# dsforza96/yocto-hair

Measured on AMD Instinct MI355X. Metric: Msamples/sec (whole node), 720x720x1536spp sphere-hairblock; per-pixel L2 vs CPU ref, higher is better.
Workload: dtype f32

## Files before the change

### include/yhair.h

```cpp
#ifndef YHAIR_H_
#define YHAIR_H_

#include <stdint.h>

#ifdef __cplusplus
extern "C" {
#endif

#define YH_OK 0
#define YH_E_INVALID -1
#define YH_E_DEVICE -2
#define YH_E_STATE -3
#define YH_E_IO -4
#define YH_E_SELFTEST -5


typedef struct yh_shape {
  int          num_vertices;
  const float* positions;
  const float* normals;
  const float* radius;
  int          num_lines;
  const int*   lines;
  int          num_triangles;
// ... 123 lines not shown
int yh_unpack_tiles_device(yh_context* ctx, const void* device_packed,
    int src_rank, int world, void* device_image);
int64_t yh_shard_pixels(const yh_context* ctx, int rank, int world);

int yh_gather_framebuffer(yh_context** contexts, int n, float* rgba);

int yh_download_rng(yh_context* ctx, uint64_t* state_inc);

int yh_trace_samples_counted(yh_context* ctx, int nsamples, yh_workcounts* out);

int yh_last_trace_ms(const yh_context* ctx, float* ms, int* launches);

int yh_launch_shape(const yh_context* ctx);
int yh_kernel_trials(const yh_context* ctx, double* ms_per_sample, int* trials, int count);
int yh_trials_pending(const yh_context* ctx);
int         yh_set_trial_cache_dir(const char* dir);
const char* yh_default_trial_cache_dir(void);

int yh_tile_costs(yh_context* ctx, uint32_t* ticks, int count);
int yh_item_costs(yh_context* ctx, uint32_t* costs, int count);


#define YH_HAIR_BRDF_FLOATS 30

enum {
  YH_LOBE_DIFFUSE            = 0,
  YH_LOBE_SPECULAR           = 1,
  YH_LOBE_METAL              = 2,
  YH_LOBE_TRANSMISSION       = 3,
  YH_LOBE_REFRACTION         = 4,
// ... 54 lines not shown
```

### yocto-hair_amd/csrc/dev_items.h

```cpp
#ifndef YH_DEV_ITEMS_H_
#define YH_DEV_ITEMS_H_
#include "dev_path.h"

using namespace yhd;

#define YH_BLOCK 512
#define YH_MIN_WAVES 4

#define YH_QUADS (YH_BLOCK / 4)
template <bool COUNT, bool GENERAL, int BLOCK, int SHADER, int MODE = YH_MODE_QUAD>
YH_DEV void trace_items(const yhd_scene& sc, const yhd_state& st, int nsamples, yhd_counters* counters, unsigned int block = blockIdx.x,
    unsigned int blocks = gridDim.x) {
  constexpr int LPP    = YH_IS_HEX(MODE) ? 16 : YH_IS_OCT(MODE) ? 8 : 4;
  constexpr int GROUPS = BLOCK / LPP;
  extern __shared__ v4f lds_dyn[];
  YH_LDS unsigned int* lds_stack = (YH_LDS unsigned int*)lds_dyn;
  YH_LDS v4f*          lds_tabs  = (YH_LDS v4f*)(lds_stack + ((MODE == YH_MODE_QUAD ? sc.stack_entries : YH_IS_HEX(MODE) ? sc.stack_entries16 : sc.stack_entries8) + YH_HITROWS) * GROUPS);
  trace_ctx tc;
  tc.sc = &sc;
  tc.ls = nullptr, tc.sc_dev = nullptr;
  YH_LDS float* lds_cam;
  stage_tables(sc, lds_tabs, threadIdx.x, blockDim.x, tc, lds_cam);
  __syncthreads();

  tc.lds_stack = lds_stack + (threadIdx.x / LPP);
  stats_t stats = {};
  tc.stats = COUNT ? &stats : nullptr;

  const int lane = threadIdx.x & 63;
  const int by_position = (int)(blocks * (BLOCK / 64));
  int       t_first     = __builtin_amdgcn_readfirstlane((int)(block * (BLOCK / 64) + (threadIdx.x >> 6)));
  while (true) {
    int t = t_first;
    if (t < 0) {
      if (lane == 0) t = atomicAdd(st.tile_cursor, 1);
      t = __builtin_amdgcn_readfirstlane(t) + by_position;
    }
    t_first = -1;
    if (t >= st.num_tiles) break;
    unsigned long long t0 = wall_clock64();
    int  item  = st.tiles[t];
    int  half  = 0;
    if (YH_IS_OCT(MODE)) half = item & 1, item >>= 1;
    if (YH_IS_HEX(MODE)) half = item & 3, item >>= 2;
    int  tile  = item >> 2, part = item & 3;
    int  pq    = YH_IS_HEX(MODE) ? half * 4 + (lane >> 4) : YH_IS_OCT(MODE) ? half * 8 + (lane >> 3) : lane >> 2;
    int  i     = (tile % st.tiles_x) * YH_TILE + (part & 1) * 4 + (pq & 3);
    int  j     = (tile / st.tiles_x) * YH_TILE + (part >> 1) * 4 + (pq >> 2);
    bool owner = i < st.width && j < st.height;
    size_t pix = owner ? (size_t)j * st.width + i : 0;
    rng_t  rng;
    rng.state      = st.rng_state[pix];
    rng.inc        = st.rng_inc[pix];
    yhd_float4 acc = st.accum[pix];
    int    left    = owner ? nsamples : 0;
    bool   alive   = false;
    path_t ps;
    ps.bounce = 0, ps.hit = false;
    unsigned long long cyc_trace = 0, cyc_shade = 0;
    unsigned int       w_iters = 0, w_steps = 0, l_steps = 0, l_iters = 0;
    while (true) {
      if (!alive && left > 0) {
        yhd_camera cam;
        for (int k = 0; k < 12; k++) cam.frame[k] = lds_cam[k];
        cam.lens = lds_cam[12], cam.film_x = lds_cam[13], cam.film_y = lds_cam[14], cam.focus = lds_cam[15], cam.aperture = lds_cam[16];
        path_begin(cam, ps, rng, i, j, st.width, st.height);
        left--;
        alive = true;
      }
      if (!__any(alive)) break;
// ... 42 lines not shown
      }
      {
        unsigned int b[10] = {stats.t_node, stats.l_node, stats.t_line, stats.l_line, stats.t_tri, stats.l_tri, stats.t_enter,
            stats.l_enter, stats.t_scene, stats.l_scene};
        for (int k = 0; k < 10; k++) {
          for (int off = 32; off > 0; off >>= 1) b[k] += (unsigned int)__shfl_xor((int)b[k], off, 64);
          if (lane == 0) atomicAdd(&counters->branch[k], (unsigned long long)b[k]);
        }
      }
      stats = stats_t{};
    }
    if (owner && (lane & (LPP - 1)) == 0) {
      st.rng_state[pix] = rng.state;
      st.accum[pix]     = acc;
    }
    if (lane == 0) {
      unsigned int dt = (unsigned int)(wall_clock64() - t0);
      if (YH_IS_OCT(MODE) || YH_IS_HEX(MODE)) atomicAdd(&st.tile_cost[item], dt);
      else st.tile_cost[item] = dt;
      if (COUNT) atomicAdd(&counters->cyc_tile, (unsigned long long)dt);
    }
  }
}
typedef void (*trace_kernel_t)(const yhd_scene, const yhd_state, int, yhd_counters*);
#define YH_OCT_BLOCK 256
template <bool COUNT, bool GENERAL, int BLOCK, int WAVES, int MODE = YH_MODE_QUAD>
__global__ __launch_bounds__(BLOCK, WAVES) void k_trace(const yhd_scene sc, const yhd_state st,
    int nsamples, yhd_counters* counters) {
  trace_items<COUNT, GENERAL, BLOCK, YH_SHADER_PATH, MODE>(sc, st, nsamples, counters);
}
template <bool GENERAL>
__global__ __launch_bounds__(YH_BLOCK, YH_MIN_WAVES) void k_trace_sbs(const yhd_scene sc, const yhd_state st, int nsamples, int oct_blocks,
    int quad_items, int oct_entries) {
  if ((int)blockIdx.x < oct_blocks) {
    yhd_state so   = st;
    so.tiles       = st.tiles + quad_items, so.num_tiles = oct_entries, so.tile_cursor = st.tile_cursor + 16;
    trace_items<false, GENERAL, YH_BLOCK, YH_SHADER_PATH, YH_MODE_OCT>(sc, so, nsamples, nullptr, blockIdx.x, (unsigned)oct_blocks);
  } else {
    yhd_state sq = st;
    sq.num_tiles = quad_items;
    trace_items<false, GENERAL, YH_BLOCK, YH_SHADER_PATH, YH_MODE_QUAD>(sc, sq, nsamples, nullptr, blockIdx.x - (unsigned)oct_blocks, gridDim.x - (unsigned)oct_blocks);
  }
}
#endif
```

### yocto-hair_amd/csrc/yh_device.h

```cpp
#ifndef YH_DEVICE_H_
#define YH_DEVICE_H_
#include <stdint.h>

#define YH_KIND_LINES 1
#define YH_KIND_TRIANGLES 2
#define YH_TILE 8
#define YH_MAX_LIGHTS 16
#define YH_MAX_ENVS 4

typedef struct yhd_float4 { float x, y, z, w; } yhd_float4;
typedef struct yhd_int4 { int x, y, z, w; } yhd_int4;

typedef struct yhd_object {
  float frame[12];
  float inv_frame[12];
  int   kind;
  int   node_base;
  int   prim_base;
  int   vert_base;
  int   elem_base;
  int   has_normals;
  int   material;
  int   has_texcoords;
  float wbox_min[4], wbox_max[4];
// ... 96 lines not shown
  const yhd_float4* light_table;
  int               light_table_f4;
  int               scene_wide_root;
  const float*      env_tab;
  int               env_tab_light;
  int               env_tab_k, env_tab_stride;
  int               lds_materials;
  int               stack_entries8;
  int               stack_entries16;
  const yhd_float4* lane_blob;
  long long         lane_blob_units;
} yhd_scene;
#define YH_MATERIAL_F4 17
#define YHD_LDS_TABLES_F4(sc) ((sc)->lds_scene_f4 + 5 + (sc)->light_table_f4 + ((sc)->env_tab_k + 3) / 4 + YH_MATERIAL_F4 * (sc)->lds_materials)

typedef struct yhd_state {
  uint64_t*   rng_state;
  uint64_t*   rng_inc;
  yhd_float4* accum;
  const int*  tiles;
  int*        tile_cursor;
  int         num_groups;
  int         group_begin[9];
  unsigned int* tile_cost;
  int         num_tiles;
  int         shader;
  int         launch_shape;
  int         width, height;
  int         tiles_x;
  int         samples_done;
  int         bounces;
  float       clamp;
  int         shard_rank, shard_world;
} yhd_state;

enum yhd_shape {
  YH_SHAPE_QUAD       = 0,
  YH_SHAPE_QUAD_DENSE = 1,
  YH_SHAPE_RETIRED    = 2,
  YH_SHAPE_STREAM     = 3,
  YH_SHAPE_OCT        = 4,
  YH_SHAPE_SBS        = 5,
  YH_SHAPE_HEX        = 6,
  YH_SHAPE_OCT_PAIRS  = 7,
  YH_SHAPE_HEX_GROUPS = 8,
  YH_SHAPES
};
enum yhd_shape_kind { YH_SHAPE_KIND_QUAD, YH_SHAPE_KIND_WIDE, YH_SHAPE_KIND_STREAM, YH_SHAPE_KIND_SBS, YH_SHAPE_KIND_RETIRED };
// ... 55 lines not shown
```

### yocto-hair_amd/host/context.cpp

```cpp
#include "context_internal.h"

std::string g_create_error = "no error";

int fail(yh_context* ctx, int code, const char* fmt, ...) {
  char    buf[512];
  va_list ap;
  va_start(ap, fmt);
  vsnprintf(buf, sizeof(buf), fmt, ap);
  va_end(ap);
  if (ctx) ctx->error = buf;
  else g_create_error = buf;
  return code;
}

int upload(yh_context* ctx, DevBuf& buf, const void* src, size_t bytes) {
  YH_WAIT(ctx);
  buf.reset();
  size_t alloc = std::max<size_t>(bytes, 16);
  HIPCHK(ctx, hipMalloc(&buf.p, alloc));
  buf.bytes = alloc;
  if (bytes) HIPCHK(ctx, hipMemcpy(buf.p, src, bytes, hipMemcpyHostToDevice));
  return YH_OK;
}
int upload_keep(yh_context* ctx, DevBuf& buf, const void* src, size_t bytes) {
// ... 69 lines not shown
  (void)hipSetDevice(ctx->device);
  if (ctx->stream && wait_for_launch(ctx) != YH_OK) return;
  if (ctx->ev0) (void)hipEventDestroy(ctx->ev0);
  if (ctx->ev1) (void)hipEventDestroy(ctx->ev1);
  if (ctx->stream) (void)hipStreamDestroy(ctx->stream);
  delete ctx;
}

const char* yh_last_error(const yh_context* ctx) { return ctx ? ctx->error.c_str() : g_create_error.c_str(); }

int yh_set_shard(yh_context* ctx, int rank, int world) {
  if (!ctx) return YH_E_INVALID;
  if (world < 1 || rank < 0 || rank >= world) return fail(ctx, YH_E_INVALID, "bad shard %d of %d", rank, world);
  if (rank != ctx->rank || world != ctx->world) ctx->item_cost.clear();
  ctx->rank = rank, ctx->world = world;
  ctx->have_state = false;
  return YH_OK;
}

int yh_image_size(const yh_context* ctx, int* width, int* height) {
  if (!ctx || !ctx->have_state) return YH_E_STATE;
  if (width) *width = ctx->state.width;
  if (height) *height = ctx->state.height;
  return YH_OK;
}

int yh_download(yh_context* ctx, float* rgba) {
  if (!ctx || !rgba) return YH_E_INVALID;
  if (!ctx->have_state) return fail(ctx, YH_E_STATE, "yh_download before yh_init_state");
  HIPCHK(ctx, hipSetDevice(ctx->device));
  size_t bytes = (size_t)ctx->state.width * ctx->state.height * 16;
// ... 44 lines not shown
```

### yocto-hair_amd/host/context_internal.h

```cpp
#ifndef YH_CONTEXT_INTERNAL_H_
#define YH_CONTEXT_INTERNAL_H_
#include <hip/hip_runtime_api.h>
#include <dlfcn.h>
#include <fcntl.h>
#include <sys/stat.h>
#include <unistd.h>
#include <rccl/rccl.h>

#include <algorithm>
#include <chrono>
#include <cmath>
#include <cstdarg>
#include <cstddef>
#include <cstdio>
#include <cstdlib>
#include <cstring>
#include <limits>
#include <map>
#include <mutex>
#include <tuple>
#include <string>
#include <memory>
#include <thread>
#include <vector>
// ... 170 lines not shown
  bool        poisoned = false;
  bool      have_scene = false;
  yhd_scene scene{};
  DevBuf    d_prims, d_vpos, d_elems, d_objects, d_materials, d_scene_nodes,
      d_scene_prims, d_light_cdf, d_env_texels, d_light_table, d_env_tab;
  int       stack_need = 0, stack_need8 = 0, stack_need16 = 0;
  struct LaneShape { int kind, num_nodes, prim_base, num_prims; long long node_off, test_off, node_off8, node_off16; };
  std::vector<LaneShape>   lane_shapes;
  long long                lane_units = 0;
  DevBuf                   d_lane_blob;
  bool             have_state = false;
  yhd_state        state{};
  yh_trace_params  params{};
  DevBuf           d_textures, d_tex_texels, d_vtex, d_maps;
  DevBuf           d_rng_state, d_rng_inc, d_accum, d_tiles, d_image, d_counters, d_tile_cursor, d_tile_cost;
  std::vector<int> owned;
  std::vector<unsigned int>  item_cost;
  int              rank = 0, world = 1;
  int              num_tiles_total = 0;
  float            last_ms = 0;
  int              last_launches = 0;
  int              last_nsamples = 0;
  unsigned         launches_of_image = 0;
  int              launch_shape = YH_SHAPE_QUAD;
  int              last_shape = -1;
  bool             async_pending = false;
  bool             last_counted = false;
  DevBuf                  d_gather_send, d_gather_recv;
  std::vector<ncclComm_t> comms;
  std::vector<int>        comm_devices;
// ... 45 lines not shown
int upload(yh_context* ctx, DevBuf& buf, const void* src, size_t bytes);
int upload_keep(yh_context* ctx, DevBuf& buf, const void* src, size_t bytes);
int alloc_zero(yh_context* ctx, DevBuf& buf, size_t bytes);
yhd_float4 node_lo(const yhh::Node& n);
yhd_float4 node_hi(const yhh::Node& n);
int forced_shape();
void trials_load(yh_context* ctx);
bool trials_off();
void record_launch(yh_context* ctx, int nsamples, bool fresh_costs);
bool trial_pending(const yh_context* ctx);
int pick_launch_shape(const yh_context* ctx, int nsamples);
bool settle_launch_shape(yh_context* ctx, bool counted, int nsamples, bool sync);
void build_work_items(const yh_context* ctx, std::vector<int>& items);
void prepare_work_list(yh_context* ctx, std::vector<int>& items, int shape);
int upload_work_items(yh_context* ctx);
int expensive_items(const yh_context* ctx, const std::vector<int>& items);
bool side_by_side_grids(const yh_context* ctx, int* oct_blocks, int* quad_blocks);
void split_items_side_by_side(yh_context* ctx, std::vector<int>& items);
void lay_out_range(const yh_context* ctx, int* items, size_t n, int wpb, int G, int block_offset = 0);
int replan_after_launch(yh_context* ctx, int nsamples);
bool lane_kernels_can_address(const yh_context* ctx);
int stream_geometry(const yh_context* ctx, int num_items, int* slots_per_wave, int* grid_blocks, int* lds_out, bool* single_generation = nullptr);
void note_stream_wave_log(yh_context* ctx, const unsigned long long* log, size_t waves);
void deal_items_for_stream(yh_context* ctx, std::vector<int>& items);
int build_bvh_device(yh_context* ctx, const std::vector<yhh::Box>& boxes, yhh::Tree& tree);
int stream_impl(yh_context* ctx, int nsamples, bool sync);
int trace_impl(yh_context* ctx, int nsamples, bool counted, bool sync);
int wait_for_launch(yh_context* ctx);
int side_by_side_impl(yh_context* ctx, int nsamples, bool sync);
void destroy_communicators(yh_context* ctx);
// ... 5 lines not shown
```

### yocto-hair_amd/host/launch_plan.cpp

```cpp
#include "context_internal.h"

#include "build_id.h"

static bool dense_by_costs(const yh_context* ctx, bool* known, bool* chain_bound = nullptr, bool* chain16 = nullptr) {
  uint64_t sum = 0, mx = 0;
  for (int t : ctx->owned)
    for (int p = 0; p < 4; p++) {
      uint64_t c = ctx->item_cost[(size_t)t * 4 + p];
      sum += c, mx = std::max(mx, c);
    }
  *known = mx != 0;
  if (mx == 0) return false;
  static const double share = std::max(1, getenv("YHAIR_DEVICE_SHARE") ? atoi(getenv("YHAIR_DEVICE_SHARE")) : 1);
  int    lds      = yhk_trace_lds_bytes(&ctx->scene, YH_SHAPE_QUAD);
  double resident = (double)ctx->num_cus * std::max(1, yhk_trace_occupancy(lds, ctx->scene.general_materials, YH_SHAPE_QUAD)) * (yhk_block_threads(YH_SHAPE_QUAD) / 64) / share;
  if (getenv("YHAIR_TIMING")) fprintf(stderr, "[yhair] launch shape: worth %.0f items, resident waves %.0f\n", (double)sum / (double)mx, resident);
  if (chain_bound) {
    const int    lds4 = yhk_trace_lds_bytes(&ctx->scene, YH_SHAPE_OCT);
    const double res4 = (double)ctx->num_cus * std::max(1, yhk_trace_occupancy(lds4, ctx->scene.general_materials, YH_SHAPE_OCT)) * (yhk_block_threads(YH_SHAPE_OCT) / 64) / share;
    *chain_bound      = 2.0 * (double)sum / (double)mx <= 1.1 * res4;
    if (chain16) *chain16 = 4.0 * (double)sum / (double)mx <= 2.5 * res4;
  }
  return (double)sum / (double)mx >= resident;
}
// ... 235 lines not shown
    for (int p = 0; p < 4; p++) {
      unsigned item = (unsigned)(t * 4 + p);
      keys.push_back(((uint64_t)(0xFFFFFFFFu - ctx->item_cost[item]) << 32) | item);
    }
  if (!keys.empty()) {
    auto mid = keys.begin() + keys.size() / 2;
    std::nth_element(keys.begin(), mid, keys.end());
    uint64_t median_cost = 0xFFFFFFFFu - (uint32_t)(*mid >> 32);
    uint64_t cut_cost    = std::min<uint64_t>(0xFFFFFFFFu, median_cost * 8 + 1);
    uint64_t cut_key     = (uint64_t)(0xFFFFFFFFu - (uint32_t)cut_cost) << 32;
    auto heavy_end = std::partition(keys.begin(), keys.end(), [&](uint64_t k) { return k < cut_key; });
    std::sort(keys.begin(), heavy_end);
  }
  items.resize(keys.size());
  for (size_t i = 0; i < keys.size(); i++) items[i] = (int)(keys[i] & 0xFFFFFFFFu);
}

int expensive_items(const yh_context* ctx, const std::vector<int>& items) {
  if (items.empty()) return 0;
  const uint64_t top = ctx->item_cost[(size_t)items[0]];
  int n = 0;
  for (int it : items) {
    if ((uint64_t)ctx->item_cost[(size_t)it] * 5 < top || top == 0) break;
    n++;
  }
  return n;
}
bool side_by_side_grids(const yh_context* ctx, int* oct_blocks, int* quad_blocks) {
  const int lds = yhk_trace_sbs_lds_bytes(&ctx->scene), occ = yhk_trace_sbs_occupancy(lds, ctx->scene.general_materials);
  if (occ < 1) return false;
// ... 71 lines not shown
  if (forced_shape() < 0) {
    const int kind = yhd_shapes[shape].kind;
    int       P = 0, grid = 0;
    if ((kind == YH_SHAPE_KIND_STREAM && !stream_geometry(ctx, (int)ctx->owned.size() * 4, &P, &grid, nullptr)) ||
        (kind == YH_SHAPE_KIND_WIDE && !counted && yhk_trace_occupancy(yhk_trace_lds_bytes(&ctx->scene, shape), general, shape) < 1))
      ctx->shape_ms[shape] = std::numeric_limits<double>::infinity(), shape = fallback(shape);
  }
  if (shape == ctx->state.launch_shape) return false;
  ctx->launch_shape = ctx->state.launch_shape = shape;
  return true;
}

int replan_after_launch(yh_context* ctx, int nsamples) {
  const unsigned li      = ++ctx->launches_of_image;
  const bool     refresh = (li & (li - 1)) == 0 || ctx->last_ms >= 50.0f || (!ctx->costs_settled && nsamples >= YH_TRIAL_SPP && ctx->state.shader == YH_SHADER_PATH);
  if (refresh) HIPCHK(ctx, hipMemcpy(ctx->item_cost.data(), ctx->d_tile_cost.p, ctx->item_cost.size() * 4, hipMemcpyDeviceToHost));
  if (refresh) ctx->last_nsamples = nsamples;
  if (refresh && ctx->last_shape == YH_SHAPE_SBS)
    for (int it : ctx->hy_oct_items) ctx->item_cost[(size_t)it] = (unsigned int)((double)ctx->item_cost[(size_t)it] * (1.0 / 1.48));
  if (ctx->state.shader == YH_SHADER_PATH && (refresh || ctx->have_costs)) record_launch(ctx, nsamples, refresh);
  if (!refresh) return YH_OK;
  return upload_work_items(ctx);
}

bool lane_kernels_can_address(const yh_context* ctx) { return (long long)ctx->lane_units * 32ll <= 0xFFFFFE00ll; }

int stream_geometry(const yh_context* ctx, int num_items, int* slots_per_wave, int* grid_blocks, int* lds_out, bool* single_generation) {
  if (!lane_kernels_can_address(ctx)) return 0;
  const int     wpb    = yhk_stream_block_threads() / 64;
  const int64_t pixels = (int64_t)num_items * 16;
  int           P      = (int)std::max<int64_t>(128, std::min<int64_t>(192, (pixels / ((int64_t)ctx->num_cus * 16) + 63) / 64 * 64));
  const bool    forced = getenv("YHAIR_ST_SLOTS") != nullptr;
  if (forced) P = std::max(64, std::min(4096, atoi(getenv("YHAIR_ST_SLOTS")) / 64 * 64));
  int lds_bytes = yhk_stream_lds_bytes(YHD_LDS_TABLES_F4(&ctx->scene), P);
// ... 144 lines not shown
```

### yocto-hair_amd/host/scene_upload.cpp

```cpp
#include "context_internal.h"

#include <atomic>

static int dev_alloc(yh_context* ctx, DevBuf& buf, size_t bytes) {
  buf.reset();
  HIPCHK(ctx, hipMalloc(&buf.p, std::max<size_t>(bytes, 16)));
  buf.bytes = std::max<size_t>(bytes, 16);
  return YH_OK;
}

void make_material(const yh_material& m, yhd_material& d) {
  memset(&d, 0, sizeof(d));
  memcpy(d.emission, m.emission, 12);
  memcpy(d.color, m.color, 12);
  float dmax    = fmax_(fmax_(m.color[0], m.color[1]), m.color[2]);
  d.diffuse_pdf = dmax ? dmax / dmax : 0.0f;
  d.thin        = m.thin;
  d.specular = m.specular, d.metallic = m.metallic, d.roughness = m.roughness, d.ior = m.ior;
  d.transmission = m.transmission;
  d.opacity      = m.opacity * ((1.0f + 1.0f + 1.0f) / 3);
  if (d.opacity > 0.999f) d.opacity = 1;
  d.emission_tex = m.emission_tex - 1, d.color_tex = m.color_tex - 1, d.scattering_tex = m.scattering_tex - 1;
  d.trdepth = m.trdepth;
  d.plain = m.specular == 0 && m.metallic == 0 && m.transmission == 0 && d.opacity == 1 && m.emission_tex == 0 &&
// ... 110 lines not shown
  std::vector<yhd_int4>   elems;
  size_t total_prim_f4 = 0;
  for (int si = 0; si < sd->num_shapes; si++) {
    auto& s = sd->shapes[si];
    if (s.num_vertices <= 0 || !s.positions) return fail(ctx, YH_E_INVALID, "shape %d has no vertices", si);
    const bool lines = s.num_lines > 0;
    if (!lines && s.num_triangles <= 0) return fail(ctx, YH_E_INVALID, "shape %d has no lines or triangles", si);
    const int nel = lines ? s.num_lines : s.num_triangles;
    if (nel >= (1 << 27)) return fail(ctx, YH_E_INVALID, "shape %d has %d elements (limit %d)", si, nel, (1 << 27) - 1);
    info[si].kind = lines ? YH_KIND_LINES : YH_KIND_TRIANGLES, info[si].num_prims = nel, info[si].has_normals = s.normals != nullptr;
    info[si].prim_base = (int)total_prim_f4;
    total_prim_f4 += (size_t)nel * (lines ? 4 : 6);
  }
  if (total_prim_f4 > (size_t)std::numeric_limits<int>::max()) return fail(ctx, YH_E_INVALID, "scene too large for 32-bit record offsets (%zu primitive float4)", total_prim_f4);
  int rc;
  ctx->have_scene = false, ctx->have_state = false;
  ctx->scene.lane_blob = nullptr, ctx->scene.prims = nullptr;
  ctx->d_prims.reset(), ctx->d_lane_blob.reset();
  if ((rc = dev_alloc(ctx, ctx->d_prims, total_prim_f4 * 16))) return rc;
  lap("validation, record array");
  const char* bvh_env   = getenv("YHAIR_BVH");
  const bool  host_only = bvh_env && !strcmp(bvh_env, "host"), device_all = bvh_env && !strcmp(bvh_env, "device");
  for (int si = 0; si < sd->num_shapes; si++) {
    auto&      s     = sd->shapes[si];
    auto&      I     = info[si];
    const bool lines = I.kind == YH_KIND_LINES;
    const int  nel   = I.num_prims;
    const int* idx   = lines ? s.lines : s.triangles;
    {
      std::atomic<bool> bad{false};
      parallel_for(nel * (lines ? 2 : 3), [&](int k) {
// ... 492 lines not shown
```

### yocto-hair_amd/host/trace_launch.cpp

```cpp
#include "context_internal.h"

int wait_for_launch(yh_context* ctx) {
  if (ctx->poisoned) return fail(ctx, YH_E_DEVICE, "a launch of this context exceeded its deadline: the context refuses further work, destroy it");
  const double timeout = yhh::launch_timeout_s();
  const int    device  = ctx->device;
  hipStream_t  stream  = ctx->stream;
  int          e       = 0;
  const double spin_s  = std::min(std::min(0.050, timeout), 1.25e-3 * (double)ctx->last_ms + 0.001);
  {
    const auto t0 = std::chrono::steady_clock::now();
    while (true) {
      const hipError_t q = hipStreamQuery(stream);
      if (q == hipSuccess) return YH_OK;
      if (q != hipErrorNotReady) return fail(ctx, YH_E_DEVICE, "hipStreamQuery: %s", hipGetErrorString(q));
      if (std::chrono::duration<double>(std::chrono::steady_clock::now() - t0).count() > spin_s) break;
    }
  }
  const int    rc      = ctx->sync_call.run(
      [device, stream]() {
        hipError_t se = hipSetDevice(device);
        return (int)(se != hipSuccess ? se : hipStreamSynchronize(stream));
      },
      timeout, &e);
  if (rc == yhh::WAIT_EXPIRED) {
// ... 56 lines not shown
    ctx->have_costs = false, ctx->costs_settled = false, ctx->dense = -1, ctx->chain = -1, ctx->chain16 = -1, ctx->launch_shape = YH_SHAPE_QUAD;
    for (double& t : ctx->shape_ms) t = 0;
    for (int& t : ctx->shape_trials) t = 0;
    new_image = true;
  }
  std::vector<int> tiles;
  build_work_items(ctx, tiles);
  const int first_shape = forced_shape() >= 0 ? forced_shape() : ctx->launch_shape;
  prepare_work_list(ctx, tiles, params->shader == YH_SHADER_PATH ? first_shape : YH_SHAPE_QUAD);
  tiles.reserve(4 * (size_t)ctx->num_tiles_total * 4 + 4);
  int rc;
  if ((rc = upload(ctx, ctx->d_rng_state, st.data(), npix * 8))) return rc;
  if ((rc = upload(ctx, ctx->d_rng_inc, inc.data(), npix * 8))) return rc;
  if ((rc = alloc_zero(ctx, ctx->d_accum, npix * 16))) return rc;
  if ((rc = alloc_zero(ctx, ctx->d_image, npix * 16))) return rc;
  {
    const size_t n = tiles.size();
    tiles.resize(std::max(n, 4 * owned.size() * 4), 0);
    if ((rc = upload(ctx, ctx->d_tiles, tiles.data(), tiles.size() * 4))) return rc;
    tiles.resize(n);
  }
  if ((rc = alloc_zero(ctx, ctx->d_counters, sizeof(yhd_counters)))) return rc;
  if ((rc = alloc_zero(ctx, ctx->d_tile_cursor, 8 * 16 * 4))) return rc;
  if ((rc = alloc_zero(ctx, ctx->d_tile_cost, (size_t)ctx->num_tiles_total * 16))) return rc;
  auto& s = ctx->state;
  s.tile_cursor = (int*)ctx->d_tile_cursor.p, s.tile_cost = (unsigned int*)ctx->d_tile_cost.p;
  s.rng_state = (uint64_t*)ctx->d_rng_state.p, s.rng_inc = (uint64_t*)ctx->d_rng_inc.p;
  s.accum = (yhd_float4*)ctx->d_accum.p, s.tiles = (const int*)ctx->d_tiles.p;
  s.launch_shape = first_shape;
  s.num_tiles = (int)tiles.size(), s.width = w, s.height = h, s.tiles_x = tx;
  if (new_image || !same_work) ctx->launches_of_image = 0;
  s.samples_done = 0, s.bounces = params->bounces, s.clamp = params->clamp, s.shader = params->shader;
  s.shard_rank = ctx->rank, s.shard_world = ctx->world;
  ctx->have_state = true;
  lap("work list, buffers, copies");
  if (new_image) trials_load(ctx);
  bool measured = false;
  for (int t : owned)
    for (int q = 0; q < 4 && !measured; q++) measured = ctx->item_cost[(size_t)t * 4 + q] != 0;
  if (!measured && !owned.empty() && params->shader == YH_SHADER_PATH && !getenv("YHAIR_NO_PROBE")) {
    ctx->state.launch_shape = YH_SHAPE_QUAD;
    int prc = trace_impl(ctx, 1, false, true);
    if (prc) return prc;
    HIPCHK(ctx, hipMemcpy(ctx->d_rng_state.p, st.data(), npix * 8, hipMemcpyHostToDevice));
    HIPCHK(ctx, hipMemsetAsync(ctx->d_accum.p, 0, npix * 16, ctx->stream));
    YH_WAIT(ctx);
    ctx->state.samples_done = 0, ctx->launches_of_image = 0, ctx->last_shape = -1, ctx->last_ms = 0, ctx->last_launches = 0;
    ctx->have_costs = true;
    lap("probe launch + plan");
  }
  return YH_OK;
}

template <typename F>
static int end_launch(yh_context* ctx, int nsamples, bool sync, F&& read_back) {
  HIPCHK(ctx, hipEventRecord(ctx->ev1, ctx->stream));
  ctx->state.samples_done += nsamples;
  ctx->last_launches = 1;
  if (!sync) return YH_OK;
  if (int wrc = wait_for_launch(ctx)) return wrc;
  HIPCHK(ctx, hipEventElapsedTime(&ctx->last_ms, ctx->ev0, ctx->ev1));
  if (int rc = read_back()) return rc;
// ... 119 lines not shown
            "results back, accept"};
        double      sum = 0;
        for (int k = 0; k < 5; k++) sum += (double)c[52 + k];
        for (int k = 0; k < 5 && c[24]; k++)
          fprintf(stderr, "[yhair]   step part %d %-46s %7.0f cycles per step (%4.1f %% of the stamped step)\n", k, part[k], (double)c[52 + k] / (double)c[24], sum > 0 ? 100.0 * (double)c[52 + k] / sum : 0.0);
      }
      const char* br[10] = {"step", "pop", "scene", "enter", "fetch", "node", "line-leaf", "tri-leaf", "push", "2nd-seg"};
      for (int b = 0; b < 10; b++)
        fprintf(stderr, "[yhair]   branch %-9s ran in %5.1f %% of the wave steps (%llu times), %.1f lanes on average\n", br[b],
            c[32] ? 100.0 * (double)c[32 + 2 * b] / (double)c[32] : 0.0, c[32 + 2 * b], c[32 + 2 * b] ? (double)c[33 + 2 * b] / (double)c[32 + 2 * b] : 0.0);
    }
    return YH_OK;
  });
}

int trace_impl(yh_context* ctx, int nsamples, bool counted, bool sync) {
  if (!ctx) return YH_E_INVALID;
  if (ctx->poisoned) return fail(ctx, YH_E_DEVICE, "a launch of this context exceeded its deadline: the context refuses further launches, destroy it");
  if (!ctx->have_state) return fail(ctx, YH_E_STATE, "yh_trace_samples before yh_init_state");
  if (nsamples < 0) return fail(ctx, YH_E_INVALID, "negative sample count");
  HIPCHK(ctx, hipSetDevice(ctx->device));
  if (nsamples == 0 || ctx->owned.empty()) {
    ctx->state.samples_done += nsamples;
    ctx->last_ms = 0, ctx->last_launches = 0;
    return YH_OK;
  }
  const bool path = ctx->state.shader == YH_SHADER_PATH;
  if (counted && !path) return fail(ctx, YH_E_INVALID, "work counters exist for the path shader only");
  if (settle_launch_shape(ctx, counted, nsamples, sync)) {
    if (int wrc = wait_for_launch(ctx)) return wrc;
    if (int rc = upload_work_items(ctx)) return rc;
  }
  const int shape = path ? ctx->state.launch_shape : YH_SHAPE_QUAD;
  ctx->last_shape = shape, ctx->last_counted = counted, ctx->planned_settled = ctx->costs_settled;
  const int kind = yhd_shapes[shape].kind;
  if (kind == YH_SHAPE_KIND_STREAM) return stream_impl(ctx, nsamples, sync);
  if (kind == YH_SHAPE_KIND_RETIRED) return fail(ctx, YH_E_INVALID, "launch shape 2 (quads over 8-wide nodes) was a developer kernel and is not built (profiles/r03/w8_oct_ab.txt)");
  if (kind == YH_SHAPE_KIND_SBS) return side_by_side_impl(ctx, nsamples, sync);
  int waves_per_block = yhk_block_threads(shape) / 64;
  int lds_bytes       = yhk_trace_lds_bytes(&ctx->scene, shape);
  const bool exact    = path && ctx->params.hair_exact && !counted;
  int occupancy       = exact ? yhk_trace_exact_occupancy(lds_bytes, ctx->scene.general_materials) : yhk_trace_occupancy(lds_bytes, ctx->scene.general_materials, shape);
  if (occupancy < 1) return fail(ctx, YH_E_DEVICE, "k_trace cannot run with %d bytes of LDS per block", lds_bytes);
  int resident        = ctx->num_cus * occupancy;
  int want            = (ctx->state.num_tiles + waves_per_block - 1) / waves_per_block;
  int grid            = std::max(1, std::min(want, resident));
  HIPCHK(ctx, hipMemsetAsync(ctx->d_tile_cursor.p, 0, 8 * 16 * 4, ctx->stream));
  HIPCHK(ctx, hipMemsetAsync(ctx->d_tile_cost.p, 0, (size_t)ctx->num_tiles_total * 16, ctx->stream));
  HIPCHK(ctx, hipEventRecord(ctx->ev0, ctx->stream));
  int e = exact ? yhk_trace_exact(&ctx->scene, &ctx->state, nsamples, lds_bytes, grid, ctx->stream)
                : yhk_trace(&ctx->scene, &ctx->state, nsamples, counted ? (yhd_counters*)ctx->d_counters.p : nullptr, shape, grid, ctx->stream);
  if (e) return fail(ctx, YH_E_DEVICE, "k_trace launch: %s", hipGetErrorString((hipError_t)e));
  return end_launch(ctx, nsamples, sync, [] { return YH_OK; });
}
int side_by_side_impl(yh_context* ctx, int nsamples, bool sync) {
  int G_o = 0, G_q = 0;
// ... 69 lines not shown
```

### yocto-hair_amd/python/yhair_capi.py

```python
import ctypes as C
import os

import numpy as np

ROOT = os.path.dirname(os.path.dirname(os.path.dirname(os.path.abspath(__file__))))
LIB_PATH = os.environ.get("YHAIR_LIB", os.path.join(ROOT, "yocto-hair_amd", "libyhair.so"))

YH_OK, YH_E_INVALID, YH_E_DEVICE, YH_E_STATE, YH_E_IO, YH_E_SELFTEST = 0, -1, -2, -3, -4, -5
YH_HAIR_BRDF_FLOATS = 30
SURFACE_BSDF_FLOATS = 29
(LOBE_DIFFUSE, LOBE_SPECULAR, LOBE_METAL, LOBE_TRANSMISSION, LOBE_REFRACTION, LOBE_DELTA_SPECULAR,
 LOBE_DELTA_METAL, LOBE_DELTA_TRANSMISSION, LOBE_DELTA_REFRACTION) = range(9)
LOBE_COUNT = 9

c_float_p = C.POINTER(C.c_float)
c_int_p = C.POINTER(C.c_int)


class Shape(C.Structure):
    _fields_ = [("num_vertices", C.c_int), ("positions", c_float_p), ("normals", c_float_p),
                ("radius", c_float_p), ("num_lines", C.c_int), ("lines", c_int_p),
                ("num_triangles", C.c_int), ("triangles", c_int_p), ("texcoords", c_float_p)]


# ... 108 lines not shown
    "yh_trace_samples_async": (C.c_int, [C.c_void_p, C.c_int]),
    "yh_synchronize": (C.c_int, [C.c_void_p]),
    "yh_download": (C.c_int, [C.c_void_p, c_float_p]),
    "yh_pack_tiles_device": (C.c_int, [C.c_void_p, C.c_void_p, C.c_int64, C.POINTER(C.c_int64)]),
    "yh_unpack_tiles_device": (C.c_int, [C.c_void_p, C.c_void_p, C.c_int, C.c_int, C.c_void_p]),
    "yh_gather_framebuffer": (C.c_int, [C.POINTER(C.c_void_p), C.c_int, c_float_p]),
    "yh_shard_pixels": (C.c_int64, [C.c_void_p, C.c_int, C.c_int]),
    "yh_download_rng": (C.c_int, [C.c_void_p, C.POINTER(C.c_uint64)]),
    "yh_trace_samples_counted": (C.c_int, [C.c_void_p, C.c_int, C.POINTER(WorkCounts)]),
    "yh_last_trace_ms": (C.c_int, [C.c_void_p, c_float_p, c_int_p]),
    "yh_launch_shape": (C.c_int, [C.c_void_p]),
    "yh_tile_costs": (C.c_int, [C.c_void_p, C.POINTER(C.c_uint32), C.c_int]),
    "yh_item_costs": (C.c_int, [C.c_void_p, C.POINTER(C.c_uint32), C.c_int]),
    "yh_kernel_trials": (C.c_int, [C.c_void_p, C.POINTER(C.c_double), C.POINTER(C.c_int), C.c_int]),
    "yh_trials_pending": (C.c_int, [C.c_void_p]),
    "yh_set_trial_cache_dir": (C.c_int, [C.c_char_p]),
    "yh_default_trial_cache_dir": (C.c_char_p, []),
    "yh_hair_brdf_batch": (C.c_int, [C.c_void_p, C.c_int, C.POINTER(Material), c_float_p,
                                     c_float_p, c_float_p, c_float_p]),
    "yh_curves_to_lines": (C.c_int, [C.c_void_p, C.c_int, c_float_p, c_float_p, c_float_p, C.c_int, c_float_p,
                                     c_float_p, c_float_p, c_int_p]),
    "yh_bvh_build_gpu": (C.c_int, [C.c_void_p, C.c_int, c_float_p, c_float_p, c_int_p]),
    "yh_bvh_build": (C.c_int, [C.c_int, c_float_p, c_float_p, c_int_p]),
    "yh_bvh_build_wide": (C.c_int, [C.c_int, c_float_p, C.c_int, c_float_p]),
    "yh_bvh_build_wide_gpu": (C.c_int, [C.c_void_p, C.c_int, c_float_p, C.c_int, c_float_p]),
    "yh_surface_lobe_batch": (C.c_int, [C.c_void_p, C.c_int, C.c_int, c_float_p, c_float_p, c_float_p, c_float_p,
                                        c_float_p, c_float_p]),
    "yh_surface_bsdf_batch": (C.c_int, [C.c_void_p, C.c_int, C.POINTER(Material), c_float_p, c_float_p, c_float_p,
                                        c_float_p, c_float_p]),
    "yh_hair_eval_batch": (C.c_int, [C.c_void_p, C.c_int, c_float_p, c_float_p, c_float_p, c_float_p]),
# ... 147 lines not shown
        out = np.zeros(tx * ty, np.uint32)
        self._chk(self.lib.yh_tile_costs(self.h, out.ctypes.data_as(C.POINTER(C.c_uint32)), len(out)))
        return out.reshape(ty, tx)

    def kernel_trials(self):
        ms, tr = (C.c_double * 16)(), (C.c_int * 16)()
        n = self.lib.yh_kernel_trials(self.h, ms, tr, 16)
        self._chk(min(n, 0))
        return {k: (round(ms[k], 5), tr[k]) for k in range(min(n, 16)) if tr[k] or ms[k]}

    def trials_pending(self):
        n = self.lib.yh_trials_pending(self.h)
        self._chk(min(n, 0))
        return n > 0

    def item_costs(self):
        w, h = C.c_int(), C.c_int()
        self._chk(self.lib.yh_image_size(self.h, C.byref(w), C.byref(h)))
        n = ((w.value + 7) // 8) * ((h.value + 7) // 8) * 4
        out = np.zeros(n, np.uint32)
        self._chk(self.lib.yh_item_costs(self.h, out.ctypes.data_as(C.POINTER(C.c_uint32)), n))
        return out

    def download(self):
        img = np.zeros((self.height, self.width, 4), np.float32)
        self._chk(self.lib.yh_download(self.h, fptr(img)))
        return img

    def download_rng(self):
        rng = np.zeros((self.height * self.width, 2), np.uint64)
# ... 80 lines not shown
```

Baseline: 2582.

## Let idle waves run ahead on expensive tiles for the next launch

```diff
diff --git a/include/yhair.h b/include/yhair.h
--- a/include/yhair.h
+++ b/include/yhair.h
@@ -161,6 +161,7 @@
 int yh_launch_shape(const yh_context* ctx);
 int yh_kernel_trials(const yh_context* ctx, double* ms_per_sample, int* trials, int count);
 int yh_trials_pending(const yh_context* ctx);
+int yh_run_ahead_stats(yh_context* ctx, long long* pixels_ahead, long long* samples_ahead, long long* samples_picked_up);
 int         yh_set_trial_cache_dir(const char* dir);
 const char* yh_default_trial_cache_dir(void);
 
diff --git a/yocto-hair_amd/csrc/dev_items.h b/yocto-hair_amd/csrc/dev_items.h
--- a/yocto-hair_amd/csrc/dev_items.h
+++ b/yocto-hair_amd/csrc/dev_items.h
@@ -8,7 +8,58 @@
 #define YH_MIN_WAVES 4
 
 #define YH_QUADS (YH_BLOCK / 4)
-template <bool COUNT, bool GENERAL, int BLOCK, int SHADER, int MODE = YH_MODE_QUAD>
+template <bool GENERAL, int GROUPS, int MODE>
+YH_DEV void run_ahead(trace_ctx& tc, const yhd_state& st, int nsamples, int t, YH_LDS float* lds_cam) {
+  constexpr int LPP = YH_IS_OCT(MODE) ? 8 : 4;
+  const int lane = threadIdx.x & 63;
+  const int cap  = nsamples / 2;
+  const unsigned int* done = st.ahead.ctl;
+  if (t < 0 || cap < 1 || __any(__hip_atomic_load(done, __ATOMIC_RELAXED, __HIP_MEMORY_SCOPE_AGENT) >= st.ahead.entries)) return;
+  __threadfence_block();
+  if (st.ahead.low_prio) __builtin_amdgcn_s_setprio(0);
+  int  item  = st.tiles[t];
+  int  half  = 0;
+  if (YH_IS_OCT(MODE)) half = item & 1, item >>= 1;
+  int  tile  = item >> 2, part = item & 3;
+  int  pq    = YH_IS_OCT(MODE) ? half * 8 + (lane >> 3) : lane >> 2;
+  int  i     = (tile % st.tiles_x) * YH_TILE + (part & 1) * 4 + (pq & 3);
+  int  j     = (tile / st.tiles_x) * YH_TILE + (part >> 1) * 4 + (pq >> 2);
+  bool owner = i < st.width && j < st.height;
+  size_t pix = owner ? (size_t)j * st.width + i : 0;
+  rng_t  rng;
+  rng.state      = st.rng_state[pix];
+  rng.inc        = st.rng_inc[pix];
+  yhd_float4 acc = st.accum[pix];
+  int    left    = owner ? cap : 0;
+  bool   alive   = false;
+  path_t ps;
+  ps.bounce = 0, ps.hit = false;
+  while (true) {
+    if (!alive && left > 0) {
+      yhd_camera cam;
+      for (int k = 0; k < 12; k++) cam.frame[k] = lds_cam[k];
+      cam.lens = lds_cam[12], cam.film_x = lds_cam[13], cam.film_y = lds_cam[14], cam.focus = lds_cam[15], cam.aperture = lds_cam[16];
+      path_begin(cam, ps, rng, i, j, st.width, st.height);
+      left--;
+      alive = true;
+    }
+    if (!__any(alive)) break;
+    if (__any(__hip_atomic_load(done, __ATOMIC_RELAXED, __HIP_MEMORY_SCOPE_AGENT) >= st.ahead.entries)) break;
+    hit_t isec;
+    if (alive) {
+      isec  = trace_ray<false, GROUPS, !GENERAL, MODE>(tc, ps.ray, -1, nullptr);
+      alive = path_step<false, GROUPS, GENERAL>(tc, ps, isec, rng, st.bounces);
+      if (!alive) {
+        path_end(ps, st.clamp, acc);
+        if ((lane & (LPP - 1)) == 0) st.ahead.rng[pix] = rng.state, st.ahead.accum[pix] = acc, st.ahead.n[pix] = cap - left;
+      }
+    }
+  }
+  int n = (lane & (LPP - 1)) == 0 && owner ? cap - left - (alive ? 1 : 0) : 0, p = n > 0 ? 1 : 0;
+  for (int off = 32; off > 0; off >>= 1) n += __shfl_xor(n, off, 64), p += __shfl_xor(p, off, 64);
+  if (lane == 0 && n > 0) atomicAdd(&st.ahead.ctl[YH_AHEAD_PIXELS], (unsigned int)p), atomicAdd(&st.ahead.ctl[YH_AHEAD_SAMPLES], (unsigned int)n);
+}
+template <bool COUNT, bool GENERAL, int BLOCK, int SHADER, int MODE = YH_MODE_QUAD, bool AHEAD = false>
 YH_DEV void trace_items(const yhd_scene& sc, const yhd_state& st, int nsamples, yhd_counters* counters, unsigned int block = blockIdx.x,
     unsigned int blocks = gridDim.x) {
   constexpr int LPP    = YH_IS_HEX(MODE) ? 16 : YH_IS_OCT(MODE) ? 8 : 4;
@@ -28,6 +79,9 @@
   tc.stats = COUNT ? &stats : nullptr;
 
   const int lane = threadIdx.x & 63;
+  const bool ahead = AHEAD && st.ahead.n != nullptr;
+  int        ahead_entry = -1;
+  if (AHEAD && ahead && st.ahead.low_prio) __builtin_amdgcn_s_setprio(1);
   const int by_position = (int)(blocks * (BLOCK / 64));
   int       t_first     = __builtin_amdgcn_readfirstlane((int)(block * (BLOCK / 64) + (threadIdx.x >> 6)));
   while (true) {
@@ -54,6 +108,23 @@
     rng.inc        = st.rng_inc[pix];
     yhd_float4 acc = st.accum[pix];
     int    left    = owner ? nsamples : 0;
+    int    most    = nsamples;
+    if (AHEAD && ahead) {
+      int picked = 0;
+      if (owner) {
+        const int an = st.ahead.n[pix];
+        if (an != 0) {
+          if ((lane & (LPP - 1)) == 0) st.ahead.n[pix] = 0;
+          if (an <= nsamples) rng.state = st.ahead.rng[pix], acc = st.ahead.accum[pix], left = nsamples - an, picked = an;
+        }
+      }
+      if (__any(picked != 0)) {
+        int m = left, s = (lane & (LPP - 1)) == 0 ? picked : 0;
+        for (int off = 32; off > 0; off >>= 1) m = max(m, __shfl_xor(m, off, 64)), s += __shfl_xor(s, off, 64);
+        most = __builtin_amdgcn_readfirstlane(m);
+        if (lane == 0) atomicAdd(&st.ahead.ctl[YH_AHEAD_PICKED], (unsigned int)s);
+      }
+    }
     bool   alive   = false;
     path_t ps;
     ps.bounce = 0, ps.hit = false;
@@ -126,12 +197,25 @@
       st.rng_state[pix] = rng.state;
       st.accum[pix]     = acc;
     }
+    unsigned int dt_scaled = 0;
+    if (AHEAD && ahead) {
+      dt_scaled = (unsigned int)(wall_clock64() - t0);
+      if (most < nsamples) dt_scaled = __builtin_amdgcn_readfirstlane((unsigned int)((float)dt_scaled * ((float)nsamples / (float)max(most, 1))));
+      if (t < by_position && dt_scaled >= st.ahead.min_ticks) ahead_entry = t;
+    }
     if (lane == 0) {
-      unsigned int dt = (unsigned int)(wall_clock64() - t0);
+      unsigned int dt = AHEAD && ahead ? dt_scaled : (unsigned int)(wall_clock64() - t0);
+      if (AHEAD && ahead) {
+        if (2 * most < nsamples) st.ahead.brief[item] = 1;
+        atomicAdd(&st.ahead.ctl[0], 1u);
+      }
       if (YH_IS_OCT(MODE) || YH_IS_HEX(MODE)) atomicAdd(&st.tile_cost[item], dt);
       else st.tile_cost[item] = dt;
       if (COUNT) atomicAdd(&counters->cyc_tile, (unsigned long long)dt);
     }
+  }
+  if constexpr (AHEAD) {
+    if (ahead) run_ahead<GENERAL, GROUPS, MODE>(tc, st, nsamples, ahead_entry, lds_cam);
   }
 }
 typedef void (*trace_kernel_t)(const yhd_scene, const yhd_state, int, yhd_counters*);
@@ -139,7 +223,7 @@
 template <bool COUNT, bool GENERAL, int BLOCK, int WAVES, int MODE = YH_MODE_QUAD>
 __global__ __launch_bounds__(BLOCK, WAVES) void k_trace(const yhd_scene sc, const yhd_state st,
     int nsamples, yhd_counters* counters) {
-  trace_items<COUNT, GENERAL, BLOCK, YH_SHADER_PATH, MODE>(sc, st, nsamples, counters);
+  trace_items<COUNT, GENERAL, BLOCK, YH_SHADER_PATH, MODE, !COUNT && !GENERAL && BLOCK == YH_BLOCK && WAVES == YH_MIN_WAVES && MODE == YH_MODE_QUAD>(sc, st, nsamples, counters);
 }
 template <bool GENERAL>
 __global__ __launch_bounds__(YH_BLOCK, YH_MIN_WAVES) void k_trace_sbs(const yhd_scene sc, const yhd_state st, int nsamples, int oct_blocks,
@@ -147,11 +231,11 @@
   if ((int)blockIdx.x < oct_blocks) {
     yhd_state so   = st;
     so.tiles       = st.tiles + quad_items, so.num_tiles = oct_entries, so.tile_cursor = st.tile_cursor + 16;
-    trace_items<false, GENERAL, YH_BLOCK, YH_SHADER_PATH, YH_MODE_OCT>(sc, so, nsamples, nullptr, blockIdx.x, (unsigned)oct_blocks);
+    trace_items<false, GENERAL, YH_BLOCK, YH_SHADER_PATH, YH_MODE_OCT, !GENERAL>(sc, so, nsamples, nullptr, blockIdx.x, (unsigned)oct_blocks);
   } else {
     yhd_state sq = st;
     sq.num_tiles = quad_items;
-    trace_items<false, GENERAL, YH_BLOCK, YH_SHADER_PATH, YH_MODE_QUAD>(sc, sq, nsamples, nullptr, blockIdx.x - (unsigned)oct_blocks, gridDim.x - (unsigned)oct_blocks);
+    trace_items<false, GENERAL, YH_BLOCK, YH_SHADER_PATH, YH_MODE_QUAD, !GENERAL>(sc, sq, nsamples, nullptr, blockIdx.x - (unsigned)oct_blocks, gridDim.x - (unsigned)oct_blocks);
   }
 }
 #endif
diff --git a/yocto-hair_amd/csrc/yh_device.h b/yocto-hair_amd/csrc/yh_device.h
--- a/yocto-hair_amd/csrc/yh_device.h
+++ b/yocto-hair_amd/csrc/yh_device.h
@@ -134,6 +134,20 @@
 #define YH_MATERIAL_F4 17
 #define YHD_LDS_TABLES_F4(sc) ((sc)->lds_scene_f4 + 5 + (sc)->light_table_f4 + ((sc)->env_tab_k + 3) / 4 + YH_MATERIAL_F4 * (sc)->lds_materials)
 
+typedef struct yhd_ahead {
+  int*          n;
+  uint64_t*     rng;
+  yhd_float4*   accum;
+  unsigned int* ctl;
+  unsigned int* brief;
+  unsigned int  entries;
+  unsigned int  min_ticks;
+  int           low_prio;
+} yhd_ahead;
+#define YH_AHEAD_PIXELS 16
+#define YH_AHEAD_SAMPLES 17
+#define YH_AHEAD_PICKED 18
+
 typedef struct yhd_state {
   uint64_t*   rng_state;
   uint64_t*   rng_inc;
@@ -152,6 +166,7 @@
   int         bounces;
   float       clamp;
   int         shard_rank, shard_world;
+  yhd_ahead   ahead;
 } yhd_state;
 
 enum yhd_shape {
diff --git a/yocto-hair_amd/host/context.cpp b/yocto-hair_amd/host/context.cpp
--- a/yocto-hair_amd/host/context.cpp
+++ b/yocto-hair_amd/host/context.cpp
@@ -107,7 +107,7 @@
   if (world < 1 || rank < 0 || rank >= world) return fail(ctx, YH_E_INVALID, "bad shard %d of %d", rank, world);
   if (rank != ctx->rank || world != ctx->world) ctx->item_cost.clear();
   ctx->rank = rank, ctx->world = world;
-  ctx->have_state = false;
+  ctx->have_state = false, ctx->ahead_stale = true;
   return YH_OK;
 }
 
diff --git a/yocto-hair_amd/host/context_internal.h b/yocto-hair_amd/host/context_internal.h
--- a/yocto-hair_amd/host/context_internal.h
+++ b/yocto-hair_amd/host/context_internal.h
@@ -208,6 +208,11 @@
   yh_trace_params  params{};
   DevBuf           d_textures, d_tex_texels, d_vtex, d_maps;
   DevBuf           d_rng_state, d_rng_inc, d_accum, d_tiles, d_image, d_counters, d_tile_cursor, d_tile_cost;
+  DevBuf           d_ahead_n, d_ahead_rng, d_ahead_accum, d_ahead_ctl;
+  bool             ahead_live = false;
+  bool             ahead_stale = false;
+  bool             last_ahead = false;
+  unsigned int     top_cost = 0;
   std::vector<int> owned;
   std::vector<unsigned int>  item_cost;
   int              rank = 0, world = 1;
@@ -283,6 +288,7 @@
 void build_work_items(const yh_context* ctx, std::vector<int>& items);
 void prepare_work_list(yh_context* ctx, std::vector<int>& items, int shape);
 int upload_work_items(yh_context* ctx);
+int ahead_begin_launch(yh_context* ctx, int shape, int nsamples, bool counted, bool exact);
 int expensive_items(const yh_context* ctx, const std::vector<int>& items);
 bool side_by_side_grids(const yh_context* ctx, int* oct_blocks, int* quad_blocks);
 void split_items_side_by_side(yh_context* ctx, std::vector<int>& items);
diff --git a/yocto-hair_amd/host/launch_plan.cpp b/yocto-hair_amd/host/launch_plan.cpp
--- a/yocto-hair_amd/host/launch_plan.cpp
+++ b/yocto-hair_amd/host/launch_plan.cpp
@@ -273,6 +273,7 @@
   }
   items.resize(keys.size());
   for (size_t i = 0; i < keys.size(); i++) items[i] = (int)(keys[i] & 0xFFFFFFFFu);
+  const_cast<yh_context*>(ctx)->top_cost = items.empty() ? 0 : ctx->item_cost[(size_t)items[0]];
 }
 
 int expensive_items(const yh_context* ctx, const std::vector<int>& items) {
@@ -374,10 +375,18 @@
 int replan_after_launch(yh_context* ctx, int nsamples) {
   const unsigned li      = ++ctx->launches_of_image;
   const bool     refresh = (li & (li - 1)) == 0 || ctx->last_ms >= 50.0f || (!ctx->costs_settled && nsamples >= YH_TRIAL_SPP && ctx->state.shader == YH_SHADER_PATH);
+  std::vector<unsigned int> prev, brief;
+  if (refresh && ctx->last_ahead) prev = ctx->item_cost;
   if (refresh) HIPCHK(ctx, hipMemcpy(ctx->item_cost.data(), ctx->d_tile_cost.p, ctx->item_cost.size() * 4, hipMemcpyDeviceToHost));
   if (refresh) ctx->last_nsamples = nsamples;
   if (refresh && ctx->last_shape == YH_SHAPE_SBS)
     for (int it : ctx->hy_oct_items) ctx->item_cost[(size_t)it] = (unsigned int)((double)ctx->item_cost[(size_t)it] * (1.0 / 1.48));
+  if (!prev.empty()) {
+    brief.resize(prev.size());
+    HIPCHK(ctx, hipMemcpy(brief.data(), (const unsigned int*)ctx->d_ahead_ctl.p + 32, brief.size() * 4, hipMemcpyDeviceToHost));
+    for (size_t k = 0; k < prev.size(); k++)
+      if (brief[k] && prev[k]) ctx->item_cost[k] = prev[k];
+  }
   if (ctx->state.shader == YH_SHADER_PATH && (refresh || ctx->have_costs)) record_launch(ctx, nsamples, refresh);
   if (!refresh) return YH_OK;
   return upload_work_items(ctx);
diff --git a/yocto-hair_amd/host/scene_upload.cpp b/yocto-hair_amd/host/scene_upload.cpp
--- a/yocto-hair_amd/host/scene_upload.cpp
+++ b/yocto-hair_amd/host/scene_upload.cpp
@@ -148,7 +148,7 @@
   }
   if (total_prim_f4 > (size_t)std::numeric_limits<int>::max()) return fail(ctx, YH_E_INVALID, "scene too large for 32-bit record offsets (%zu primitive float4)", total_prim_f4);
   int rc;
-  ctx->have_scene = false, ctx->have_state = false;
+  ctx->have_scene = false, ctx->have_state = false, ctx->ahead_stale = true;
   ctx->scene.lane_blob = nullptr, ctx->scene.prims = nullptr;
   ctx->d_prims.reset(), ctx->d_lane_blob.reset();
   if ((rc = dev_alloc(ctx, ctx->d_prims, total_prim_f4 * 16))) return rc;
diff --git a/yocto-hair_amd/host/trace_launch.cpp b/yocto-hair_amd/host/trace_launch.cpp
--- a/yocto-hair_amd/host/trace_launch.cpp
+++ b/yocto-hair_amd/host/trace_launch.cpp
@@ -94,6 +94,11 @@
   if ((rc = upload(ctx, ctx->d_rng_inc, inc.data(), npix * 8))) return rc;
   if ((rc = alloc_zero(ctx, ctx->d_accum, npix * 16))) return rc;
   if ((rc = alloc_zero(ctx, ctx->d_image, npix * 16))) return rc;
+  if ((rc = alloc_zero(ctx, ctx->d_ahead_n, npix * 4))) return rc;
+  if ((rc = alloc_zero(ctx, ctx->d_ahead_rng, npix * 8))) return rc;
+  if ((rc = alloc_zero(ctx, ctx->d_ahead_accum, npix * 16))) return rc;
+  if ((rc = alloc_zero(ctx, ctx->d_ahead_ctl, 32 * 4 + (size_t)ctx->num_tiles_total * 16))) return rc;
+  ctx->ahead_live = false, ctx->ahead_stale = false, ctx->last_ahead = false;
   {
     const size_t n = tiles.size();
     tiles.resize(std::max(n, 4 * owned.size() * 4), 0);
@@ -112,6 +117,7 @@
   if (new_image || !same_work) ctx->launches_of_image = 0;
   s.samples_done = 0, s.bounces = params->bounces, s.clamp = params->clamp, s.shader = params->shader;
   s.shard_rank = ctx->rank, s.shard_world = ctx->world;
+  s.ahead = yhd_ahead{};
   ctx->have_state = true;
   lap("work list, buffers, copies");
   if (new_image) trials_load(ctx);
@@ -126,6 +132,7 @@
     HIPCHK(ctx, hipMemsetAsync(ctx->d_accum.p, 0, npix * 16, ctx->stream));
     YH_WAIT(ctx);
     ctx->state.samples_done = 0, ctx->launches_of_image = 0, ctx->last_shape = -1, ctx->last_ms = 0, ctx->last_launches = 0;
+    ctx->last_ahead = false;
     ctx->have_costs = true;
     lap("probe launch + plan");
   }
@@ -275,6 +282,43 @@
   });
 }
 
+constexpr bool YH_RUN_AHEAD_DEFAULT = true;
+int ahead_begin_launch(yh_context* ctx, int shape, int nsamples, bool counted, bool exact) {
+  const char* env = getenv("YHAIR_RUN_AHEAD");
+  const bool  on  = (env ? atoi(env) != 0 : YH_RUN_AHEAD_DEFAULT) && ctx->state.shader == YH_SHADER_PATH && !counted && !exact && !ctx->scene.general_materials && (shape == YH_SHAPE_QUAD || shape == YH_SHAPE_SBS) &&
+                   nsamples >= 2 * YH_TRIAL_SPP && !trial_pending(ctx) && ctx->top_cost > 0 && ctx->d_ahead_n.p;
+  if (ctx->ahead_live && (!on || ctx->ahead_stale)) {
+    HIPCHK(ctx, hipMemsetAsync(ctx->d_ahead_n.p, 0, ctx->d_ahead_n.bytes, ctx->stream));
+    ctx->ahead_live = false;
+  }
+  ctx->ahead_stale = false, ctx->last_ahead = on;
+  ctx->state.ahead = yhd_ahead{};
+  if (!on) return YH_OK;
+  HIPCHK(ctx, hipMemsetAsync(ctx->d_ahead_ctl.p, 0, ctx->d_ahead_ctl.bytes, ctx->stream));
+  yhd_ahead& a = ctx->state.ahead;
+  a.n = (int*)ctx->d_ahead_n.p, a.rng = (uint64_t*)ctx->d_ahead_rng.p, a.accum = (yhd_float4*)ctx->d_ahead_accum.p;
+  a.ctl = (unsigned int*)ctx->d_ahead_ctl.p, a.brief = a.ctl + 32;
+  a.entries = (unsigned int)ctx->state.num_tiles;
+  a.min_ticks = (unsigned int)std::min(4.0e9, std::max(1.0, (double)ctx->top_cost / 5.0 * (double)nsamples / (double)std::max(1, ctx->last_nsamples)));
+  a.low_prio  = getenv("YHAIR_RUN_AHEAD_PRIO") && atoi(getenv("YHAIR_RUN_AHEAD_PRIO")) != 0;
+  ctx->ahead_live = true;
+  return YH_OK;
+}
+int yh_run_ahead_stats(yh_context* ctx, long long* pixels_ahead, long long* samples_ahead, long long* samples_picked_up) {
+  if (!ctx) return YH_E_INVALID;
+  if (!ctx->have_state) return fail(ctx, YH_E_STATE, "yh_run_ahead_stats before yh_init_state");
+  unsigned int c[32] = {};
+  if (ctx->last_ahead) {
+    HIPCHK(ctx, hipSetDevice(ctx->device));
+    YH_WAIT(ctx);
+    HIPCHK(ctx, hipMemcpy(c, ctx->d_ahead_ctl.p, sizeof(c), hipMemcpyDeviceToHost));
+  }
+  if (pixels_ahead) *pixels_ahead = c[YH_AHEAD_PIXELS];
+  if (samples_ahead) *samples_ahead = c[YH_AHEAD_SAMPLES];
+  if (samples_picked_up) *samples_picked_up = c[YH_AHEAD_PICKED];
+  return YH_OK;
+}
+
 int trace_impl(yh_context* ctx, int nsamples, bool counted, bool sync) {
   if (!ctx) return YH_E_INVALID;
   if (ctx->poisoned) return fail(ctx, YH_E_DEVICE, "a launch of this context exceeded its deadline: the context refuses further launches, destroy it");
@@ -295,12 +339,13 @@
   const int shape = path ? ctx->state.launch_shape : YH_SHAPE_QUAD;
   ctx->last_shape = shape, ctx->last_counted = counted, ctx->planned_settled = ctx->costs_settled;
   const int kind = yhd_shapes[shape].kind;
+  const bool exact = path && ctx->params.hair_exact && !counted;
+  if (int rc = ahead_begin_launch(ctx, shape, nsamples, counted, exact)) return rc;
   if (kind == YH_SHAPE_KIND_STREAM) return stream_impl(ctx, nsamples, sync);
   if (kind == YH_SHAPE_KIND_RETIRED) return fail(ctx, YH_E_INVALID, "launch shape 2 (quads over 8-wide nodes) was a developer kernel and is not built (profiles/r03/w8_oct_ab.txt)");
   if (kind == YH_SHAPE_KIND_SBS) return side_by_side_impl(ctx, nsamples, sync);
   int waves_per_block = yhk_block_threads(shape) / 64;
   int lds_bytes       = yhk_trace_lds_bytes(&ctx->scene, shape);
-  const bool exact    = path && ctx->params.hair_exact && !counted;
   int occupancy       = exact ? yhk_trace_exact_occupancy(lds_bytes, ctx->scene.general_materials) : yhk_trace_occupancy(lds_bytes, ctx->scene.general_materials, shape);
   if (occupancy < 1) return fail(ctx, YH_E_DEVICE, "k_trace cannot run with %d bytes of LDS per block", lds_bytes);
   int resident        = ctx->num_cus * occupancy;
diff --git a/yocto-hair_amd/python/yhair_capi.py b/yocto-hair_amd/python/yhair_capi.py
--- a/yocto-hair_amd/python/yhair_capi.py
+++ b/yocto-hair_amd/python/yhair_capi.py
@@ -146,6 +146,7 @@
     "yh_item_costs": (C.c_int, [C.c_void_p, C.POINTER(C.c_uint32), C.c_int]),
     "yh_kernel_trials": (C.c_int, [C.c_void_p, C.POINTER(C.c_double), C.POINTER(C.c_int), C.c_int]),
     "yh_trials_pending": (C.c_int, [C.c_void_p]),
+    "yh_run_ahead_stats": (C.c_int, [C.c_void_p, C.POINTER(C.c_longlong), C.POINTER(C.c_longlong), C.POINTER(C.c_longlong)]),
     "yh_set_trial_cache_dir": (C.c_int, [C.c_char_p]),
     "yh_default_trial_cache_dir": (C.c_char_p, []),
     "yh_hair_brdf_batch": (C.c_int, [C.c_void_p, C.c_int, C.POINTER(Material), c_float_p,
@@ -323,6 +324,11 @@
         self._chk(min(n, 0))
         return n > 0
 
+    def run_ahead_stats(self):
+        a, b, c = C.c_longlong(), C.c_longlong(), C.c_longlong()
+        self._chk(self.lib.yh_run_ahead_stats(self.h, C.byref(a), C.byref(b), C.byref(c)))
+        return a.value, b.value, c.value
+
     def item_costs(self):
         w, h = C.c_int(), C.c_int()
         self._chk(self.lib.yh_image_size(self.h, C.byref(w), C.byref(h)))
```

After: 2441. -5.5%, worse.
